# Signalsmith-Audio/signalsmith-stretch

Hardware: AMD Instinct MI355X
Metric: Msamples/sec (in+out) at 48kHz stereo presetDefault (higher is better)
Workload: dtype f32

## Files before the change

signalsmith-stretch_amd/csrc/smst_fft.hip:

```cpp
#include "smst_kernels_common.h"
#include <type_traits>

namespace smst {

template <int SIGN> __device__ __forceinline__ fc mulTwiddle(fc v, fc w) { return fmul<(SIGN > 0)>(v, w); }
template <int SIGN> __device__ __forceinline__ fc addJ(fc a, fc b) { return (SIGN < 0) ? fsubI(a, b) : faddI(a, b); }
template <int SIGN> __device__ __forceinline__ fc subJ(fc a, fc b) { return (SIGN < 0) ? faddI(a, b) : fsubI(a, b); }
template <int SIGN> __device__ __forceinline__ fc mulJ(fc a) { return (SIGN < 0) ? fmake(a.y, -a.x) : fmake(-a.y, a.x); }

template <int SIGN>
__device__ __forceinline__ void dft4(fc &a, fc &b, fc &c, fc &d) {
	const fc apc = fadd(a, c), amc = fsub(a, c), bpd = fadd(b, d), bmd = fsub(b, d);
	a = fadd(apc, bpd);
	b = addJ<SIGN>(amc, bmd);
	c = fsub(apc, bpd);
	d = subJ<SIGN>(amc, bmd);
}
template <int SIGN>
__device__ __forceinline__ void dft4J(fc &a, fc &b, fc &c, fc &d) {
	const fc apc = addJ<SIGN>(a, c), amc = subJ<SIGN>(a, c), bpd = fadd(b, d), bmd = fsub(b, d);
	a = fadd(apc, bpd);
	b = addJ<SIGN>(amc, bmd);
	c = fsub(apc, bpd);
	d = subJ<SIGN>(amc, bmd);
// ... 91 lines not shown
	}
	return reinterpret_cast<float2 *>(src);
}

template <int SIGN>
__device__ __forceinline__ fc mulConst(fc v, float re, float im) {
	const float s = (SIGN < 0) ? -im : im;
	return fmake(v.x*re - v.y*s, v.x*s + v.y*re);
}
template <int SIGN>
__device__ __forceinline__ void dft16(fc (&v)[16]) {
#pragma unroll
	for (int i = 0; i < 4; ++i) dft4<SIGN>(v[i], v[i + 4], v[i + 8], v[i + 12]);
	const float c1 = 0.92387953251128675613f, s1 = 0.38268343236508977173f, h = 0.70710678118654752440f;
	v[1 + 4] = mulConst<SIGN>(v[1 + 4], c1, s1);
	v[1 + 8] = mulConst<SIGN>(v[1 + 8], h, h);
	v[1 + 12] = mulConst<SIGN>(v[1 + 12], s1, c1);
	v[2 + 4] = mulConst<SIGN>(v[2 + 4], h, h);
	v[2 + 12] = mulConst<SIGN>(v[2 + 12], -h, h);
	v[3 + 4] = mulConst<SIGN>(v[3 + 4], s1, c1);
	v[3 + 8] = mulConst<SIGN>(v[3 + 8], -h, h);
	v[3 + 12] = mulConst<SIGN>(v[3 + 12], -c1, -s1);
#pragma unroll
	for (int e = 0; e < 4; ++e) {
		if (e == 2) dft4J<SIGN>(v[4*e], v[4*e + 1], v[4*e + 2], v[4*e + 3]);
		else dft4<SIGN>(v[4*e], v[4*e + 1], v[4*e + 2], v[4*e + 3]);
	}
}
template <int SIGN, int RA, int N>
__device__ __forceinline__ void dftPow2(fc (&v)[N], int base, int stride) {
	if constexpr (RA == 2) {
		const fc a = v[base], b = v[base + stride];
		v[base] = fadd(a, b);
		v[base + stride] = fsub(a, b);
	} else if constexpr (RA == 4) {
		dft4<SIGN>(v[base], v[base + stride], v[base + 2*stride], v[base + 3*stride]);
	} else {
		static_assert(RA == 8, "radix 2, 4 or 8");
		fc e0 = v[base], e1 = v[base + 2*stride], e2 = v[base + 4*stride], e3 = v[base + 6*stride];
		fc o0 = v[base + stride], o1 = v[base + 3*stride], o2 = v[base + 5*stride], o3 = v[base + 7*stride];
		dft4<SIGN>(e0, e1, e2, e3);
		dft4<SIGN>(o0, o1, o2, o3);
		const float h = 0.70710678118654752440f;
		o1 = mulConst<SIGN>(o1, h, h);
		o3 = mulConst<SIGN>(o3, -h, h);
		v[base] = fadd(e0, o0); v[base + 4*stride] = fsub(e0, o0);
		v[base + stride] = fadd(e1, o1); v[base + 5*stride] = fsub(e1, o1);
		v[base + 2*stride] = addJ<SIGN>(e2, o2); v[base + 6*stride] = subJ<SIGN>(e2, o2);
		v[base + 3*stride] = fadd(e3, o3); v[base + 7*stride] = fsub(e3, o3);
	}
}
template <int R3> struct LastStage {
	static constexpr int G = (R3%3 == 0) ? 3 : 5;
	static constexpr int RA = R3/G;
	static_assert(R3%G == 0 && (RA == 2 || RA == 4 || RA == 8), "last stage: {2,4,8} x {3,5} points");
};
template <int SIGN, int R3>
__device__ __forceinline__ void dftLast(fc (&v)[R3]) {
	constexpr int G = LastStage<R3>::G, RA = LastStage<R3>::RA;
#pragma unroll
	for (int i = 0; i < G; ++i) dftPow2<SIGN, RA>(v, i, G);
#pragma unroll
	for (int i = 1; i < G; ++i) {
#pragma unroll
		for (int e = 1; e < RA; ++e) {
			const float ang = 6.28318530717958647692f*float(i*e)/float(R3);
			v[i + G*e] = mulConst<SIGN>(v[i + G*e], __builtin_cosf(ang), __builtin_sinf(ang));
		}
	}
#pragma unroll
	for (int e = 0; e < RA; ++e) {
		if constexpr (G == 3) dft3<SIGN>(v[G*e], v[G*e + 1], v[G*e + 2]);
		else dft5<SIGN>(v[G*e], v[G*e + 1], v[G*e + 2], v[G*e + 3 < R3 ? G*e + 3 : 0], v[G*e + 4 < R3 ? G*e + 4 : 0]);
	}
}

struct BlockSync { __device__ __forceinline__ void operator()() const { __syncthreads(); } };
struct NoHook { __device__ __forceinline__ void operator()() const {} };
struct NoArrival { __device__ __forceinline__ fc operator()(fc v, int) const { return v; } };
template <int FRAMES> struct FrameSet { fc f[FRAMES]; };
struct StageTwiddles { float4 w[8]; };
struct TwiddlesFromTable {};
template <int SIGN, int R3, bool LEAN, int ROUNDS = 0, int FRAMES = 1, typename Load, typename Prep, typename Store, typename Sync = BlockSync, typename LastRead = NoHook,
          typename Requested = NoHook, typename FirstWritten = NoHook, typename Arrived = NoArrival, typename TwRegs = TwiddlesFromTable>
__device__ __forceinline__ void fftFast(float2 *lds2, const float4 *__restrict__ twA, const float4 *__restrict__ twB, Load load, Prep prep, Store store,
                                        const int t = threadIdx.x, Sync sync = Sync(), LastRead lastRead = LastRead(), Requested requested = Requested(),
                                        FirstWritten firstWritten = FirstWritten(), Arrived arrived = Arrived(), TwRegs twRegs = TwRegs()) {
	static_assert(FRAMES == 1 || FRAMES == 2, "one frame, or two in lockstep");
	constexpr int MA = 16*R3, BUF = 17*MA;
	constexpr bool TW_REGS = std::is_same<TwRegs, StageTwiddles>::value;
	static_assert(!(TW_REGS && LEAN), "the lean tables have no register form");
	fc *lds = reinterpret_cast<fc *>(lds2);
	auto prepOf = [&](int j, int idx, int f) { if constexpr (FRAMES == 1) return prep(j, idx); else return prep(j, idx, f); };
	auto storeOf = [&](int j, fc u, auto r, int idx, int f) { if constexpr (FRAMES == 1) store(j, u, r, idx); else store(j, u, r, idx, f); };
	fc v[FRAMES][16];
	if (t < MA) {
#pragma unroll
		for (int k = 0; k < 16; ++k) {
			if constexpr (FRAMES == 1) v[0][k] = load(t + MA*k, k);
			else {
				const FrameSet<FRAMES> both = load(t + MA*k, k);
#pragma unroll
				for (int f = 0; f < FRAMES; ++f) v[f][k] = both.f[f];
			}
		}
	}
	requested();
	if (t < MA) {
#pragma unroll
		for (int f = 0; f < FRAMES; ++f) {
#pragma unroll
			for (int k = 0; k < 16; ++k) {
				if constexpr (FRAMES == 1) v[f][k] = arrived(v[f][k], t + MA*k);
				else v[f][k] = arrived(v[f][k], t + MA*k, k, f);
			}
		}
		fc w[16];
		if constexpr (LEAN) {
			const float4 a = twA[t], b = twA[MA + t], c = twA[2*MA + t];
			w[1] = fmake(a.x, a.y); w[2] = fmake(a.z, a.w); w[3] = fmake(b.x, b.y); w[4] = fmake(b.z, b.w);
			w[8] = fmake(c.x, c.y); w[12] = fmake(c.z, c.w);
#pragma unroll
			for (int hi = 4; hi <= 12; hi += 4) {
#pragma unroll
				for (int lo = 1; lo < 4; ++lo) w[hi + lo] = fmul<false>(w[hi], w[lo]);
			}
		} else {
			float4 wA[8];
#pragma unroll
			for (int i = 0; i < 8; ++i) {
				if constexpr (TW_REGS) wA[i] = twRegs.w[i];
				else wA[i] = twA[i*MA + t];
			}
#pragma unroll
			for (int n = 1; n < 16; ++n) {
				const float4 pr = wA[(n - 1) >> 1];
				w[n] = ((n - 1) & 1) ? fmake(pr.z, pr.w) : fmake(pr.x, pr.y);
			}
		}
#pragma unroll
		for (int f = 0; f < FRAMES; ++f) dft16<SIGN>(v[f]);
#pragma unroll
		for (int f = 0; f < FRAMES; ++f) {
#pragma unroll
			for (int pos = 0; pos < 16; ++pos) {
				const int n = (pos >> 2) + 4*(pos & 3);
				lds[f*BUF + 17*t + n] = n > 0 ? mulTwiddle<SIGN>(v[f][pos], w[n]) : v[f][pos];
			}
		}
	}
	firstWritten();
	sync();
	const int p = t >> 4, q0 = t & 15;
	if (t < MA) {
#pragma unroll
		for (int f = 0; f < FRAMES; ++f) {
#pragma unroll
			for (int k = 0; k < 16; ++k) v[f][k] = lds[f*BUF + q0 + 17*(p + R3*k)];
		}
	}
	sync();
	if (t < MA) {
		float4 wB[8];
#pragma unroll
		for (int i = 0; i < 8; ++i) wB[i] = twB[i*R3 + p];
#pragma unroll
		for (int f = 0; f < FRAMES; ++f) dft16<SIGN>(v[f]);
#pragma unroll
		for (int f = 0; f < FRAMES; ++f) {
#pragma unroll
			for (int pos = 0; pos < 16; ++pos) {
				const int n = (pos >> 2) + 4*(pos & 3);
				fc val = v[f][pos];
				if (n > 0) {
					const float4 pr = wB[(n - 1) >> 1];
					val = mulTwiddle<SIGN>(val, ((n - 1) & 1) ? fmake(pr.z, pr.w) : fmake(pr.x, pr.y));
				}
				lds[f*BUF + q0 + 256*p + 16*n] = val;
			}
		}
	}
	sync();
	if (t < 256) {
		constexpr int G = LastStage<R3>::G, RA = LastStage<R3>::RA;
		fc u[FRAMES][R3];
#pragma unroll
		for (int f = 0; f < FRAMES; ++f) {
#pragma unroll
			for (int k = 0; k < R3; ++k) u[f][k] = lds[f*BUF + t + 256*k];
		}
		lastRead();
		constexpr int CHUNK = ROUNDS ? R3/ROUNDS : (R3 <= 12 ? R3 : (R3 == 24 ? 6 : 5));
		decltype(prepOf(0, 0, 0)) ready[FRAMES][CHUNK];
#pragma unroll
		for (int f = 0; f < FRAMES; ++f) {
#pragma unroll
			for (int i = 0; i < CHUNK; ++i) {
				const int e = i/G, c = i - G*e;
				ready[f][i] = prepOf(t + 256*(e + RA*c), e + RA*c, f);
			}
		}
#pragma unroll
		for (int f = 0; f < FRAMES; ++f) dftLast<SIGN, R3>(u[f]);
#pragma unroll
		for (int f = 0; f < FRAMES; ++f) {
#pragma unroll
			for (int p0 = 0; p0 < R3; p0 += CHUNK) {
				if (p0 > 0) {
#pragma unroll
					for (int i = 0; i < CHUNK; ++i) {
						const int pos = p0 + i, e = pos/G, c = pos - G*e;
						if (pos < R3) ready[f][i] = prepOf(t + 256*(e + RA*c), e + RA*c, f);
					}
				}
#pragma unroll
				for (int i = 0; i < CHUNK; ++i) {
					const int pos = p0 + i, e = pos/G, c = pos - G*e;
					if (pos < R3) storeOf(t + 256*(e + RA*c), u[f][pos], ready[f][i], e + RA*c, f);
				}
			}
		}
	}
}

constexpr int fastBlockThreads(int R3) { return 16*R3 > 256 ? 16*R3 : 256; }

__device__ __forceinline__ bool hopWantsAnalysis(const HopDesc &hd, int which) {
	return (hd.flags & HOP_ACTIVE) && (hd.flags & HOP_NEW_SPECTRUM) && !(hd.flags & HOP_PREANALYSED) && (!which || (hd.flags & HOP_REANALYSE_PREV));
}

// ... 14 lines not shown
	if (slot > 0) r = make_float2(fmaf(xi, w.z, r.x), fmaf(xi, w.w, r.y));
	return r;
}
__device__ __forceinline__ float2 analysisSamples(const float *x0, const float *x1, int m, int slot) {
	return make_float2(slot < 15 ? x0[m] : 0.f, slot > 0 ? x1[m] : 0.f);
}
__device__ __forceinline__ float2 analysisElement(float4 w, const float *x0, const float *x1, int m, int slot) {
	const float2 x = analysisSamples(x0, x1, m, slot);
	return analysisElement(w, x.x, x.y, slot);
}
__device__ __forceinline__ fc leanModulation(float2 hb, int k, int per) {
	const float ang = 3.14159265358979323846f*float(k)/float(per);
	return fmulExpr(fpack(hb), fmake(__builtin_cosf(ang), -__builtin_sinf(ang)));
}
__device__ __forceinline__ void storeWindowed(float *dst, int m, fc u, fc tw, float wRe, float wIm, int B, int H) {
	const int halfB = B/2;
	const fc v = fmulc(u, tw);
	if (m < B - halfB) dst[m + halfB] = (2*v.x)*wRe;
	if (m >= H - halfB) dst[m - H + halfB] = (2*v.y)*wIm;
}
__device__ __forceinline__ void storeWindowed(float *dst, int m, fc u, float4 r, int B, int H) {
	storeWindowed(dst, m, u, fmake(r.x, r.y), r.z, r.w, B, H);
}

template <int R3, bool LEAN>
__global__ __launch_bounds__(fastBlockThreads(R3)) __attribute__((amdgpu_waves_per_eu(4, 4))) void kAnalyseFast(DevBatch d, IoArgs io, int sBase, int hopBase, int lateOnly) {
	extern __shared__ __attribute__((aligned(16))) unsigned char smemRaw[];
	float2 *lds = reinterpret_cast<float2 *>(smemRaw);
	const BlockCoord bc = xcdAwareBlock();
	const int k = bc.x;
	const int c = bc.y >> 1;
	const int which = bc.y & 1;
	const int s = bc.s;
	const HopDesc hd = d.hops[(size_t)(sBase + s)*d.hopStride + hopBase + k];
	if (!hopWantsAnalysis(hd, which)) return;
	if (lateOnly && analysisWindowInCall(d.B, d.M, d.I, hd.inputOffset, which, io.inSamples[sBase + s])) return;
	const int B = d.B, H = d.M, halfB = B/2, N = d.N;
	const int base = hd.inputOffset - (which ? d.I : 0) - B;
	const float *x = io.in + (size_t)(sBase + s)*io.inStreamStride + (size_t)c*io.inChannelStride;
	const float *hist = d.hist + ((size_t)(sBase + s)*d.C + c)*(size_t)d.histPitch + d.histBase[d.histCur][sBase + s] + d.histLen;
	const float2 *__restrict__ winA = d.winA, *__restrict__ winB = d.winB;
	float2 *dst = (which ? d.Xprev : d.Xcur) + rowOf(d, s, k, c);
	auto prep = [](int, int) { return 0; };
	auto store = [&](int j, fc u, int, int) { storeHalfBin(dst, j, u, H, N); };
	constexpr int MA = 16*R3;
	const float4 *__restrict__ twA = LEAN ? d.twA6 : d.twA4;
	const float2 *__restrict__ win2 = d.win2;
	const float2 hb = LEAN ? d.halfTw[min((int)threadIdx.x, MA - 1)] : make_float2(0.f, 0.f);
	if (base >= 0 && H - halfB == MA && B - halfB == 15*MA) {
		const float *x0 = x + base + halfB, *x1 = x + base - H + halfB;
		const float4 *__restrict__ win4 = d.win4;
		fftFast<-1, R3, LEAN>(lds, twA, d.twB4,
			[&](int m, int slot) {
				if constexpr (LEAN) {
					const float2 w = win2[m];
					float2 z = make_float2(0.f, 0.f);
					if (slot < 15) z.x = x0[m]*w.x;
					if (slot > 0) z.y = x1[m]*w.y;
					return fmul<false>(fpack(z), leanModulation(hb, slot, 32));
				} else {
					return fpack(analysisElement(win4[m], x0, x1, m, slot));
				}
			}, prep, store);
		return;
	}
	fftFast<-1, R3, LEAN>(lds, twA, d.twB4,
		[&](int m, int slot) {
			float xr = 0, xi = 0;
			if (m < B - halfB) { int src = base + m + halfB; xr = (src >= 0) ? x[src] : hist[src]; }
			if (m >= H - halfB) { int src = base + m - H + halfB; xi = (src >= 0) ? x[src] : hist[src]; }
			if constexpr (LEAN) {
				const float2 w = win2[m];
				return fmul<false>(fmake(xr*w.x, xi*w.y), leanModulation(hb, slot, 32));
			} else {
				const float2 a = winA[m], b = winB[m];
				return fmake(fmaf(xi, b.x, xr*a.x), fmaf(xi, b.y, xr*a.y));
			}
		}, prep, store);
}

struct TeamSync {
	volatile int *word;
	int *generation;
	__device__ __forceinline__ void operator()() const {
		asm volatile("" ::: "memory");
		__builtin_amdgcn_wave_barrier();
		if ((threadIdx.x & 63) == 0) (void)__hip_atomic_fetch_add(const_cast<int *>(word), 1, __ATOMIC_RELAXED, __HIP_MEMORY_SCOPE_WORKGROUP);
		*generation += 4;
		while (__hip_atomic_load(const_cast<int *>(word), __ATOMIC_RELAXED, __HIP_MEMORY_SCOPE_WORKGROUP) < *generation) __builtin_amdgcn_s_sleep(1);
		__builtin_amdgcn_wave_barrier();
		asm volatile("" ::: "memory");
	}
};
template <int R3, int TEAMS, int FRAMES = 1>
struct TeamWorkgroup {
	static_assert(16*R3 <= 256, "a team is 256 threads");
	static constexpr int MA = 16*R3, H = 256*R3;
	float4 *table, *twA, *twB;
	float2 *lds;
	int team, t;
	volatile int *word;
	int generation = 0;
	__device__ __forceinline__ TeamWorkgroup(unsigned char *smem, const DevBatch &d, const float4 *__restrict__ source) {
		team = __builtin_amdgcn_readfirstlane(threadIdx.x >> 8);
		t = threadIdx.x & 255;
		table = reinterpret_cast<float4 *>(smem);
		twA = table + H;
		twB = twA + (FRAMES == 1 ? 8*MA : 0);
		lds = reinterpret_cast<float2 *>(twB + 8*R3) + (size_t)team*FRAMES*(H + H/16);
		volatile int *words = reinterpret_cast<volatile int *>(reinterpret_cast<float2 *>(twB + 8*R3) + (size_t)TEAMS*FRAMES*(H + H/16));
		for (int i = threadIdx.x; i < H; i += blockDim.x) table[i] = source[i];
		if constexpr (FRAMES == 1) {
			for (int i = threadIdx.x; i < 8*MA; i += blockDim.x) twA[i] = d.twA4[i];
		} else {
			twA = nullptr;
		}
		for (int i = threadIdx.x; i < 8*R3; i += blockDim.x) twB[i] = d.twB4[i];
		if (threadIdx.x < 16) words[threadIdx.x] = 0;
		__syncthreads();
		word = words + team;
	}
	TeamWorkgroup(const TeamWorkgroup &) = delete;
	__device__ __forceinline__ TeamSync sync() { return TeamSync{word, &generation}; }
};

template <int R3, int TEAMS, bool EXACT>
__global__ __launch_bounds__(256*TEAMS) void kAnalyseTeams(DevBatch d, IoArgs io, const HopDesc *__restrict__ hopTable, int sBase, int hopBase, int tileHops, int nStreams) {
	extern __shared__ __attribute__((aligned(16))) unsigned char smemRaw[];
	constexpr int MA = 16*R3, H = 256*R3, N = 2*H;
	const int B = EXACT ? 480*R3 : d.B, halfB = B/2;
	const int total = tileHops*2*d.C*nStreams;
	TeamWorkgroup<R3, TEAMS> wg(smemRaw, d, d.win4);
	const TeamSync sync = wg.sync();
	const int t = wg.t, tA = t < MA ? t : 0;
	const int stride = gridDim.x*TEAMS;
	for (int lin = blockIdx.x + gridDim.x*wg.team; lin < total; lin += stride) {
		const BlockCoord bc = xcdAwareCoord(lin, tileHops, 2*d.C, nStreams);
		const HopDesc hd = hopTable[(size_t)(sBase + bc.s)*d.hopStride + hopBase + bc.x];
		const int c = bc.y >> 1, which = bc.y & 1;
		if (!hopWantsAnalysis(hd, which) || !analysisWindowInCall(B, H, d.I, hd.inputOffset, which, io.inSamples[sBase + bc.s])) continue;
		const int base = hd.inputOffset - (which ? d.I : 0) - B;
		const float *x = io.in + (size_t)(sBase + bc.s)*io.inStreamStride + (size_t)c*io.inChannelStride;
		const float *x0 = x + base + halfB, *x1 = x + base - H + halfB;
		float2 *dst = (which ? d.Xprev : d.Xcur) + rowOf(d, bc.s, bc.x, c);
		fftFast<-1, R3, false>(wg.lds, wg.twA, wg.twB,
			[&](int m, int slot) { return fpack(analysisElement(wg.table[tA + MA*slot], x0, x1, m, slot)); },
			[](int, int) { return 0; },
			[&](int j, fc u, int, int) { storeHalfBin(dst, j, u, H, N); }, t, sync);
		sync();
	}
}

template <int R3, bool EXACT, bool TWIST>
__global__ __launch_bounds__(512) __attribute__((amdgpu_waves_per_eu(2, 2))) void kAnalyseTeamPairs(DevBatch d, IoArgs io, const HopDesc *__restrict__ hopTable, const int *__restrict__ inSamples, int sBase, int hopBase, int tileHops, int nStreams) {
	extern __shared__ __attribute__((aligned(16))) unsigned char smemRaw[];
	constexpr int TEAMS = 2, MA = 16*R3, H = 256*R3, N = 2*H;
	const int B = EXACT ? 480*R3 : d.B, halfB = B/2;
	const int jobs = tileHops*2*d.C;
	const int passes = (jobs + 1)/2, total = passes*nStreams;
	static_assert((H + 8*R3)*sizeof(float4) + TEAMS*2*(H + H/16)*sizeof(float2) + 64 <= 160*1024, "the window, the second-stage twiddles, four transform buffers and the barrier words fit a CU's LDS (155,200 bytes at R3 = 12)");
	TeamWorkgroup<R3, TEAMS, 2> wg(smemRaw, d, d.win4);
	const TeamSync sync = wg.sync();
	const int t = wg.t, tA = t < MA ? t : 0;
	StageTwiddles twA;
#pragma unroll
	for (int i = 0; i < 8; ++i) twA.w[i] = d.twA4[i*MA + tA];
	float2 rotOf[TWIST ? R3 : 1];
	if constexpr (TWIST) {
#pragma unroll
		for (int i = 0; i < R3; ++i) rotOf[i] = d.rot[halfBinIndex(t + 256*i, H, N)];
	}
	const int stride = gridDim.x*TEAMS, rowPasses = TWIST ? tileHops : (tileHops + 1)/2;
	const int turn = 8*((((rowPasses - stride/8)%(2*rowPasses)) + 2*rowPasses)%(2*rowPasses));
	const int place = blockIdx.x + gridDim.x*wg.team;
	for (int round = 0; round*stride < total; ++round) {
		const int lin = round*stride + (place + round*turn)%stride;
		if (lin >= total) continue;
		const BlockCoord pc = xcdAwareCoord(lin, passes, 1, nStreams);
		const int nIn = inSamples[sBase + pc.s];
		HopDesc hd[2];
		BlockCoord bc[2];
		bool have[2];
#pragma unroll
		for (int f = 0; f < 2; ++f) {
			const int job = 2*pc.x + f;
			have[f] = job < jobs;
			const int j = have[f] ? job : 2*pc.x;
			if constexpr (TWIST) {
				const int c = pc.x/tileHops;
				have[f] = true;
				bc[f].y = 2*c + f;
				bc[f].x = pc.x - c*tileHops;
			} else {
				bc[f].y = j/tileHops;
				bc[f].x = j - bc[f].y*tileHops;
			}
			bc[f].s = pc.s;
			hd[f] = hopTable[(size_t)(sBase + pc.s)*d.hopStride + hopBase + bc[f].x];
		}
		const float *x0[2], *x1[2];
		float2 *dst[2];
		bool on[2];
#pragma unroll
		for (int f = 0; f < 2; ++f) {
			const int c = bc[f].y >> 1, which = bc[f].y & 1;
			const bool wanted = hopWantsAnalysis(hd[f], which), inCall = analysisWindowInCall(B, H, d.I, hd[f].inputOffset, which, nIn);
			on[f] = have[f] & wanted & inCall;
			const int base = hd[f].inputOffset - (which ? d.I : 0) - B;
			const float *x = io.in + (size_t)(sBase + pc.s)*io.inStreamStride + (size_t)c*io.inChannelStride;
			x0[f] = x + base + halfB;
			x1[f] = x + base - H + halfB;
			dst[f] = (which ? d.Xprev : d.Xcur) + rowOf(d, pc.s, bc[f].x, c);
		}
		if (!on[0] && !on[1]) continue;
		auto prep = [](int, int, int = 0) { return 0; };
		if (on[0] && on[1]) {
			float4 win[16];
			[[maybe_unused]] fc landed[TWIST ? R3 : 1];
			fftFast<-1, R3, false, 0, 2>(wg.lds, nullptr, wg.twB,
				[&](int m, int slot) {
					FrameSet<2> r;
#pragma unroll
					for (int f = 0; f < 2; ++f) r.f[f] = fpack(analysisSamples(x0[f], x1[f], m, slot));
					return r;
				},
				prep, [&](int j, fc u, int, int idx, int f) {
					if constexpr (TWIST) {
						const fc landedValue = fconjIf(u, 2*j >= H);
						float2 *row = dst[f] + halfBinIndex(j, H, N);
						if (f == 0) { landed[idx] = landedValue; *reinterpret_cast<fc *>(row) = landedValue; }
						else *row = prevHopTwist(funpack(landed[idx]), funpack(landedValue), rotOf[idx]);
					} else {
						storeHalfBin(dst[f], j, u, H, N);
					}
				}, t, sync, NoHook(),
				[&]() {
#pragma unroll
					for (int slot = 0; slot < 16; ++slot) win[slot] = wg.table[tA + MA*slot];
					asm volatile("" ::: "memory");
				},
				NoHook(), [&](fc x, int, int slot, int) { return fpack(analysisElement(win[slot], x.x, x.y, slot)); }, twA);
		} else {
			const int f = on[0] ? 0 : 1;
			const float *xa = x0[f], *xb = x1[f];
			float2 *dstOne = dst[f];
			fftFast<-1, R3, false>(wg.lds, nullptr, wg.twB,
				[&](int m, int slot) { return fpack(analysisElement(wg.table[tA + MA*slot], xa, xb, m, slot)); },
				prep, [&](int j, fc u, int, int) { storeHalfBin(dstOne, j, u, H, N); }, t, sync, NoHook(), NoHook(), NoHook(), NoArrival(), twA);
		}
		sync();
	}
}

__global__ __launch_bounds__(256) void kTwistRows(DevBatch d, IoArgs io, int sBase, int hopBase, int teams) {
	const int k = blockIdx.x, c = blockIdx.y, s = blockIdx.z;
	const HopDesc hd = d.hops[(size_t)(sBase + s)*d.hopStride + hopBase + k];
	if (!hopWantsAnalysis(hd, 1)) return;
	const int nIn = io.inSamples[sBase + s];
	if (teams && analysisWindowInCall(d.B, d.M, d.I, hd.inputOffset, 0, nIn) && analysisWindowInCall(d.B, d.M, d.I, hd.inputOffset, 1, nIn)) return;
	const float2 *cur = d.Xcur + rowOf(d, s, k, c);
	float2 *prev = d.Xprev + rowOf(d, s, k, c);
	for (int b = threadIdx.x; b < d.M; b += blockDim.x) prev[b] = prevHopTwist(cur[b], prev[b], d.rot[b]);
}

template <int R3, bool LEAN>
__global__ __launch_bounds__(fastBlockThreads(R3)) void kSynthFast(DevBatch d, int sBase, int hopBase) {
	extern __shared__ __attribute__((aligned(16))) unsigned char smemRaw[];
	float2 *lds = reinterpret_cast<float2 *>(smemRaw);
	const int k = blockIdx.x, c = blockIdx.y, s = blockIdx.z;
	const HopDesc hd = d.hops[(size_t)(sBase + s)*d.hopStride + hopBase + k];
	if (!(hd.flags & HOP_ACTIVE)) return;
	const int B = d.B, H = d.M, N = d.N;
	const float2 *X = d.OUT + rowOf(d, s, k, c);
	float *__restrict__ frame = frameOf(d, s, k, c);
	auto loadBin = [&](int j, int) { return loadHalfBin(X, j, H, N); };
	if constexpr (LEAN) {
		const float2 *__restrict__ win2 = d.win2;
		const float2 hb = d.halfTw[min((int)threadIdx.x, 255)];
		fftFast<+1, R3, true>(lds, d.twA6, d.twB4, loadBin,
			[&](int m, int) { return win2[m]; },
			[&](int m, fc u, float2 w, int j) { storeWindowed(frame, m, u, leanModulation(hb, j, 2*R3), w.x, w.y, B, H); });
	} else {
		const float4 *__restrict__ synTab = d.synTab;
		fftFast<+1, R3, false>(lds, d.twA4, d.twB4, loadBin,
			[&](int m, int) {
				return synTab[m];
			},
			[&](int m, fc u, float4 r, int) { storeWindowed(frame, m, u, r, B, H); });
	}
}

template <int R3, int TEAMS>
__global__ __launch_bounds__(256*TEAMS) void kSynthTeams(DevBatch d, const HopDesc *__restrict__ hopTable, int sBase, int hopBase, int tileHops, int nStreams) {
	extern __shared__ __attribute__((aligned(16))) unsigned char smemRaw[];
	constexpr int H = 256*R3, N = 2*H;
	const int B = d.B;
	const int total = tileHops*d.C*nStreams;
	TeamWorkgroup<R3, TEAMS> wg(smemRaw, d, d.synTab);
	const TeamSync sync = wg.sync();
	const int stride = gridDim.x*TEAMS;
	for (int lin = blockIdx.x + gridDim.x*wg.team; lin < total; lin += stride) {
		const BlockCoord bc = xcdAwareCoord(lin, tileHops, d.C, nStreams);
		const HopDesc hd = hopTable[(size_t)(sBase + bc.s)*d.hopStride + hopBase + bc.x];
		if (!(hd.flags & HOP_ACTIVE)) continue;
		const float2 *X = d.OUT + rowOf(d, bc.s, bc.x, bc.y);
		float *__restrict__ frame = frameOf(d, bc.s, bc.x, bc.y);
		fftFast<+1, R3, false>(wg.lds, wg.twA, wg.twB,
			[&](int j, int) { return loadHalfBin(X, j, H, N); },
			[&](int m, int) { return wg.table[m]; },
			[&](int m, fc u, float4 r, int) { storeWindowed(frame, m, u, r, B, H); }, wg.t, sync);
		sync();
	}
}

__device__ __forceinline__ float carriedSumAt(const DevBatch &d, size_t row, int i) { return i < d.carryLen ? loadCarrySum(d, d.carryCur, row + i) : 0.0f; }
__device__ __forceinline__ float carriedProductAt(const DevBatch &d, const float *__restrict__ carryWpOld, int i) { return i < d.carryLen ? carryWpOld[i] : 1e-30f; }
struct FrameRange { int lo, hi; };
__device__ __forceinline__ FrameRange coveringFrames(int relFirst, int relLast, int B, int I, int hopCount) {
	FrameRange r;
	r.hi = (relLast >= 0) ? relLast/I : -1;
	r.lo = (relFirst - B + 1 > 0) ? (relFirst - B + 1 + I - 1)/I : 0;
	if (r.hi > hopCount - 1) r.hi = hopCount - 1;
	return r;
}
__device__ __forceinline__ float windowProductAt(const DevBatch &d, const EmitDesc &ed, const float *__restrict__ carryWpOld, int i) {
	float wp = carriedProductAt(d, carryWpOld, i);
	if (ed.hopCount > 0) {
		const int rel = ed.nLo + i - ed.firstHopPos - d.delta;
		const FrameRange q = coveringFrames(rel, rel, d.B, d.I, ed.hopCount);
		for (int k = q.lo; k <= q.hi; ++k) wp += d.wprod[rel - k*d.I];
	}
	return wp;
}
// ... 88 lines not shown
		float *outHops = io.out + (size_t)sg*io.outStreamStride + (size_t)c*io.outChannelStride + firstHopPos;
		const float *wpHead = d.wpHead + (size_t)sg*d.wpHeadLen + off;
		auto overlapAdd = [&]() {
			float e[QN][SLOTS];
			int tt = t;
			keepUnconditional(tt);
#pragma unroll
			for (int a = 0; a < QN; ++a) {
#pragma unroll
				for (int slot = 0; slot < SLOTS; ++slot) {
					if (GI && (256*slot >= GI || a*GI + 256*slot >= GB)) continue;
					e[a][slot] = ex[inFrame(a, slot) ? a*I + 256*slot + tt : 0];
				}
			}
#pragma unroll
			for (int a = 0; a < QN; ++a) {
#pragma unroll
				for (int slot = 0; slot < SLOTS; ++slot) {
					if (GI && (256*slot >= GI || a*GI + 256*slot >= GB)) continue;
					keepUnconditional(e[a][slot]);
					acc[a + DQ][slot] = inFrame(a, slot) ? acc[a + DQ][slot] + e[a][slot] : acc[a + DQ][slot];
				}
			}
		};
		auto moveRing = [&]() {
#pragma unroll
			for (int u = 0; u + 1 < NI; ++u) {
#pragma unroll
				for (int slot = 0; slot < SLOTS; ++slot) acc[u][slot] = acc[u + 1][slot];
			}
#pragma unroll
			for (int slot = 0; slot < SLOTS; ++slot) acc[NI - 1][slot] = 0.0f;
		};
		auto productsOf = [&](int q, float (&wp)[SLOTS]) {
#pragma unroll
			for (int slot = 0; slot < SLOTS; ++slot) wp[slot] = steady[slot];
			if (q < NI) {
				Async4 head[SLOTS];
				const float *from = wpHead + q*I;
#pragma unroll
				for (int slot = 0; slot < SLOTS; ++slot) asyncLoad4(head[slot], from + (inInterval(slot) ? 256*slot + t : 0));
				asyncWait<0>();
#pragma unroll
				for (int slot = 0; slot < SLOTS; ++slot) {
					asyncArrived(head[slot]);
					if (inInterval(slot)) wp[slot] = asyncValue(head[slot]);
				}
			}
		};
		auto emitFinal = [&](int q) {
			float wp[SLOTS];
			productsOf(q, wp);
			float *to = outHops + q*I;
#pragma unroll
			for (int slot = 0; slot < SLOTS; ++slot) {
				if (inInterval(slot)) to[256*slot + t] = acc[0][slot]/wp[slot];
			}
			moveRing();
		};
		Async8 next[16];
#pragma unroll
		for (int k = 0; k < 16; ++k) asyncClear(next[k]);
		auto request = [&](int q) {
			const float2 *X = spectra + (unsigned)q*hopPitch;
			if (t < MA) {
#pragma unroll
				for (int k = 0; k < 16; ++k) asyncLoad8(next[k], X + halfBinIndex(t + MA*k, H, N));
			}
		};
		auto landed = [&]() {
			asyncWait<0>();
#pragma unroll
			for (int k = 0; k < 16; ++k) asyncArrived(next[k]);
		};
		request(0);
		landed();
		for (int q = 0; q < cnt; ++q) {
			fftFast<+1, R3, false, 2>(lds, wg.twA, wg.twB,
				[&](int, int k) { return fpack(asyncValue(next[k])); },
				[&](int m, int) { return wg.table[m]; },
				[&](int m, fc u, float4 r, int) { storeWindowed(ex, m, u, r, B, H); }, t, sync, sync,
				[&]() {
					if (q > 0) overlapAdd();
					sync();
				},
				[&]() {
					if (q > 0) emitFinal(q - 1);
					request(q + 1 < cnt ? q + 1 : q);
				},
				[&](fc v, int j) { return fconjIf(v, 2*j >= H); });
			sync();
			landed();
		}
		overlapAdd();
		sync();
		int sgE = sg, cE = c;
		keepUnconditional(sgE);
		keepUnconditional(cE);
		const SynthEmitEdge e = synthEmitEdge(d, io, __builtin_amdgcn_readfirstlane(sgE), __builtin_amdgcn_readfirstlane(cE), tileIndex);
		auto emitEdge = [&](int q) {
			float wp[SLOTS];
			productsOf(q, wp);
			const int n0 = firstHopPos + q*I;
#pragma unroll
			for (int slot = 0; slot < SLOTS; ++slot) {
				if (inInterval(slot)) synthEmitPlace(d, e, n0 + 256*slot + t, acc[0][slot], wp[slot]);
			}
			moveRing();
		};
		emitEdge(cnt - 1);
		const bool trailing = SPLIT && firstHopPos + cnt*I < e.ed.nHi;
		if (trailing) emitEdge(cnt);
		const int n0 = firstHopPos + (cnt + (trailing ? 1 : 0))*I;
#pragma unroll
		for (int u = 0; u < NI; ++u) {
#pragma unroll
			for (int slot = 0; slot < SLOTS; ++slot) {
				if (inInterval(slot)) synthEmitPlace(d, e, n0 + u*I + 256*slot + t, acc[u][slot], 1.0f);
			}
		}
	}
}

__global__ __launch_bounds__(256) void kEnergy(DevBatch d, IoArgs io, int sBase, float *__restrict__ energyOut) {
	const int s = blockIdx.x, part = blockIdx.y, parts = gridDim.y;
	if (part == 0 && (int)threadIdx.x >= parts && (int)threadIdx.x < kEnergyParts) energyOut[(size_t)(sBase + s)*kEnergyParts + threadIdx.x] = 0.0f;
	const int n = io.inSamples[sBase + s];
	const int lo = (int)((long long)n*part/parts), hi = (int)((long long)n*(part + 1)/parts);
	float acc = 0;
	for (int c = 0; c < d.C; ++c) {
		const float *x = io.in + (size_t)(sBase + s)*io.inStreamStride + (size_t)c*io.inChannelStride;
		for (int i = lo + threadIdx.x; i < hi; i += blockDim.x) {
			float v = x[i];
			acc += v*v;
		}
	}
	extern __shared__ __attribute__((aligned(16))) unsigned char smemRaw[];
	float *red = reinterpret_cast<float *>(smemRaw);
	red[threadIdx.x] = acc;
	__syncthreads();
	for (int w = 128; w > 0; w >>= 1) {
		if ((int)threadIdx.x < w) red[threadIdx.x] += red[threadIdx.x + w];
		__syncthreads();
	}
	if (threadIdx.x == 0) energyOut[(size_t)(sBase + s)*kEnergyParts + part] = red[0];
}

template <bool BIG>
__global__ __launch_bounds__(256) void kAnalyse(DevBatch d, IoArgs io, int sBase, int hopBase) {
	extern __shared__ __attribute__((aligned(16))) unsigned char smemRaw[];
	float2 *bufA = reinterpret_cast<float2 *>(smemRaw);
	float2 *bufB = bufA + d.M;

	const BlockCoord bc = xcdAwareBlock();
	const int k = bc.x;
	const int c = bc.y >> 1;
	const int which = bc.y & 1;
	const int s = bc.s;
	const HopDesc hd = d.hops[(size_t)(sBase + s)*d.hopStride + hopBase + k];
	if (!hopWantsAnalysis(hd, which)) return;

	const int B = d.B, H = d.M, halfB = B/2;
	const int base = hd.inputOffset - (which ? d.I : 0) - B;
	const float *x = io.in + (size_t)(sBase + s)*io.inStreamStride + (size_t)c*io.inChannelStride;
	const float *hist = d.hist + ((size_t)(sBase + s)*d.C + c)*(size_t)d.histPitch + d.histBase[d.histCur][sBase + s];
	const float *__restrict__ win = d.window;
	float2 *dst = (which ? d.Xprev : d.Xcur) + rowOf(d, s, k, c);
	if (BIG) bufB = dst;

	for (int m = threadIdx.x; m < H; m += blockDim.x) {
		float re = 0, im = 0;
		if (m < B - halfB) {
			int i = m + halfB;
			int src = base + i;
			float v = (src >= 0) ? x[src] : hist[d.histLen + src];
// ... 88 lines not shown
				sum[0] += f[k].x; sum[1] += f[k].y; sum[2] += f[k].z; sum[3] += f[k].w;
				wp[0] += w[k].x; wp[1] += w[k].y; wp[2] += w[k].z; wp[3] += w[k].w;
			} else if (q <= qHi) {
				const float *frame = frameOf(d, s, q, c);
#pragma unroll
				for (int j = 0; j < 4; ++j) {
					const int idx = idx0 + j;
					if (idx >= 0 && idx < B) { sum[j] += frame[idx]; wp[j] += d.wprod[idx]; }
				}
			}
		}
		for (int q = qLo + KMAX; q <= qHi; ++q) {
			const int idx0 = rel0 - q*I;
			const float *frame = frameOf(d, s, q, c);
#pragma unroll
			for (int j = 0; j < 4; ++j) {
				const int idx = idx0 + j;
				if (idx >= 0 && idx < B) { sum[j] += frame[idx]; wp[j] += d.wprod[idx]; }
			}
		}
	}
	float *out = io.out + (size_t)sg*io.outStreamStride + (size_t)c*io.outChannelStride + ed.nLo;
	if (i0 + 3 < span) {
		*reinterpret_cast<float4 *>(out + i0) = make_float4(sum[0]/wp[0], sum[1]/wp[1], sum[2]/wp[2], sum[3]/wp[3]);
	} else {
#pragma unroll
		for (int j = 0; j < 4; ++j) {
			const int i = i0 + j;
			if (i < span) {
				out[i] = sum[j]/wp[j];
			} else if (i < total) {
				storeCarrySum(d, d.carryCur ^ 1, carryRow + (i - span), sum[j]);
				if (c == 0) d.carryWp[d.carryCur ^ 1][carryWpRow(d, sg) + (i - span)] = wp[j];
			}
		}
	}
}

__global__ __launch_bounds__(256) void kEmitCarried(DevBatch d, IoArgs io) {
	const int sg = blockIdx.x;
	const EmitDesc ed = d.emit[(size_t)sg*d.emitStride];
	const int span = ed.nHi - ed.nLo, from = d.carryBase[d.carryCur][sg];
	const float *wpRow = d.carryWp[d.carryCur] + carryWpRow(d, sg) + from;
	for (int c = 0; c < d.C; ++c) {
		const size_t row = carrySumRow(d, sg, c) + from;
		float *out = io.out + (size_t)sg*io.outStreamStride + (size_t)c*io.outChannelStride + ed.nLo;
		for (int i = threadIdx.x; i < span; i += blockDim.x) {
			out[i] = carriedSumAt(d, row, i)/carriedProductAt(d, wpRow, i);
		}
	}
	__syncthreads();
	if (threadIdx.x == 0) d.carryBase[d.carryCur][sg] = from + span;
}

void launchEnergy(const DevBatch &d, const IoArgs &io, int sBase, int nStreams, int maxSamples, float *energyOut, hipStream_t st) {
	const int parts = std::max(1, std::min(kEnergyParts, maxSamples/1024));
	hipLaunchKernelGGL(kEnergy, dim3(nStreams, parts), dim3(256), 256*sizeof(float), st, d, io, sBase, energyOut);
}
template <int... R3S, typename F>
static bool withR3(int M, F f) { return M%256 == 0 && withInt<R3S...>(M/256, f); }
template <typename F> static bool withFastR3(int M, F f) { return withR3<10, 12, 20, 24>(M, f); }
template <typename F> static bool withTeamR3(int M, F f) { return withR3<10, 12>(M, f); }
static size_t fastLdsBytes(int M) { return ((size_t)M + M/16)*sizeof(float2); }
static size_t teamLdsBytes(int M, int teams, int frames = 1) {
	const size_t twA = frames == 1 ? M/2 : 0;
	return ((size_t)M + twA + M/32)*sizeof(float4) + teams*frames*fastLdsBytes(M) + 64;
}
static bool fastApplies(const DevBatch &d) { return !d.noFastFft && isFastSize(d.M); }
static bool teamsAvailable(const DevBatch &d) { return fastApplies(d) && withTeamR3(d.M, [](auto) {}) && d.fftTeams && !d.fftLean; }
static bool teamsApply(const DevBatch &d, int jobs) { return teamsAvailable(d) && (d.fftTeams == 2 || jobs >= 6*d.teamsGrid); }
static bool analysePairsApply(const DevBatch &d) { return d.analysePairs != 0; }
static int pairWorkgroups(const DevBatch &d, int passes) {
	return std::max(8, std::min((passes + 1)/2/8*8, d.teamsGrid));
}
static int teamsWorkgroups(const DevBatch &d, int jobs) {
	return std::max(8, std::min((jobs + 2)/3/8*8, d.teamsGrid));
}
constexpr int synthEmitQN(int R3) { return R3 == 10 ? 3 : 4; }
constexpr int synthEmitSlots(int R3) { return R3 == 10 ? 8 : 6; }

bool analyseTwistApplies(const DevBatch &d, int nStreams, int tileHops) { return teamsApply(d, tileHops*d.C*2*nStreams) && analysePairsApply(d); }

void launchAnalyse(const DevBatch &d, const IoArgs &io, int sBase, int nStreams, int hopBase, int tileHops, bool anyInCall, bool anyLate, hipStream_t st, bool twisted, int lateHops) {
	const dim3 grid(tileHops, d.C*2, nStreams);
	const int jobs = tileHops*d.C*2*nStreams;
	const bool teams = anyInCall && teamsApply(d, jobs);
	if (teams) {
		const WindowPad pad = windowPad(d.B, d.M);
		const bool pairs = analysePairsApply(d);
		const int passes = (tileHops*d.C*2 + 1)/2*nStreams;
		withTeamR3(d.M, [&](auto r3) { withFlag(pad.lo == 0 && pad.hi == 0, [&](auto exact) {
			if (pairs && twisted) hipLaunchKernelGGL((kAnalyseTeamPairs<r3.value, exact.value, true>), dim3(pairWorkgroups(d, passes)), dim3(512), teamLdsBytes(d.M, 2, 2), st, d, io, d.hops, io.inSamples, sBase, hopBase, tileHops, nStreams);
			else if (pairs) hipLaunchKernelGGL((kAnalyseTeamPairs<r3.value, exact.value, false>), dim3(pairWorkgroups(d, passes)), dim3(512), teamLdsBytes(d.M, 2, 2), st, d, io, d.hops, io.inSamples, sBase, hopBase, tileHops, nStreams);
			else hipLaunchKernelGGL((kAnalyseTeams<r3.value, 3, exact.value>), dim3(teamsWorkgroups(d, jobs)), dim3(768), teamLdsBytes(d.M, 3), st, d, io, d.hops, sBase, hopBase, tileHops, nStreams);
		}); });
		countLaunch(LK_ANALYSE_TEAMS);
		if (pairs) countLaunch(LK_ANALYSE_PAIRS);
		if (pairs && twisted) countLaunch(LK_ANALYSE_TWIST);
		if (!anyLate) return;
	}
	auto twistRows = [&] {
		if (!twisted || lateHops <= 0) return;
		hipLaunchKernelGGL(kTwistRows, dim3(std::min(lateHops, tileHops), d.C, nStreams), dim3(256), 0, st, d, io, sBase, hopBase, teams ? 1 : 0);
		countLaunch(LK_TWIST_ROWS);
	};
	const int lateOnly = teams ? 1 : 0;
	countLaunch(fastApplies(d) ? LK_ANALYSE_FAST : LK_ANALYSE_GENERIC);
	if (!d.noFastFft && withFastR3(d.M, [&](auto r3) { withFlag(d.fftLean != 0, [&](auto lean) {
			hipLaunchKernelGGL((kAnalyseFast<r3.value, lean.value>), grid, dim3(fastBlockThreads(r3.value)), fastLdsBytes(d.M), st, d, io, sBase, hopBase, lateOnly);
		}); })) { twistRows(); return; }
	size_t lds = 2*(size_t)d.M*sizeof(float2);
	if (fftNeedsScratch(d.M)) hipLaunchKernelGGL(kAnalyse<true>, grid, dim3(256), lds/2, st, d, io, sBase, hopBase);
	else hipLaunchKernelGGL(kAnalyse<false>, grid, dim3(256), lds, st, d, io, sBase, hopBase);
	twistRows();
}
void launchSynth(const DevBatch &d, int sBase, int nStreams, int hopBase, int tileHops, hipStream_t st) {
	const dim3 grid(tileHops, d.C, nStreams);
	const int jobs = tileHops*d.C*nStreams;
	if (teamsApply(d, jobs)) {
		withTeamR3(d.M, [&](auto r3) {
			hipLaunchKernelGGL((kSynthTeams<r3.value, 3>), dim3(teamsWorkgroups(d, jobs)), dim3(768), teamLdsBytes(d.M, 3), st, d, d.hops, sBase, hopBase, tileHops, nStreams);
		});
		countLaunch(LK_SYNTH_TEAMS);
		return;
	}
	countLaunch(fastApplies(d) ? LK_SYNTH_FAST : LK_SYNTH_GENERIC);
	if (!d.noFastFft && withFastR3(d.M, [&](auto r3) { withFlag(d.fftLean != 0, [&](auto lean) {
			hipLaunchKernelGGL((kSynthFast<r3.value, lean.value>), grid, dim3(fastBlockThreads(r3.value)), fastLdsBytes(d.M), st, d, sBase, hopBase);
		}); })) return;
	size_t lds = 2*(size_t)d.M*sizeof(float2);
	if (fftNeedsScratch(d.M)) hipLaunchKernelGGL(kSynth<true>, grid, dim3(256), lds/2, st, d, sBase, hopBase);
	else hipLaunchKernelGGL(kSynth<false>, grid, dim3(256), lds, st, d, sBase, hopBase);
}
bool synthEmitApplies(const DevBatch &d, int nStreams, int tileHops) {
	if (!teamsAvailable(d) || !d.synthEmit) return false;
	if (!(d.delta == 0 || d.delta == d.I)) return false;
	const int QN = synthEmitQN(d.M/256), SLOTS = synthEmitSlots(d.M/256);
	if (QN*d.I < d.B || d.I > 256*SLOTS || d.B > d.N) return false;
	if ((QN + 2)*d.I > d.wpHeadLen) return false;
	return d.synthEmit == 2 || (tileHops >= 8 && nStreams*d.C >= 64);
}
void launchEmitProducts(const DevBatch &d, int sBase, int nStreams, int tileIndex, hipStream_t st) {
	hipLaunchKernelGGL(kEmitProducts, dim3(divUp(d.wpHeadLen + d.carryLen, 256), nStreams), dim3(256), 0, st, d, sBase, tileIndex);
}
template <int GI, int GB> struct SynthEmitGeometry { static constexpr int interval = GI, block = GB, slots = (GI + 255)/256; };
template <int R3, typename F>
static void withSynthEmitGeometry(const DevBatch &d, F f) {
	using Slots = std::integral_constant<int, synthEmitSlots(R3)>;
	auto is = [&](auto g) { return d.I == g.interval && d.B == g.block && (f(g, std::integral_constant<int, g.slots>()), true); };
	if constexpr (R3 == 12) { if (is(SynthEmitGeometry<1440, 5760>()) || is(SynthEmitGeometry<1323, 5292>())) return; }
	if constexpr (R3 == 10) { if (is(SynthEmitGeometry<1920, 4800>()) || is(SynthEmitGeometry<1764, 4410>())) return; }
	f(SynthEmitGeometry<0, 0>(), Slots());
}
void launchSynthEmit(const DevBatch &d, const IoArgs &io, int sBase, int nStreams, int tileIndex, hipStream_t st) {
	const int items = nStreams*d.C;
	const int wgs = std::min(divUp(items, 2), d.teamsGrid);
	withTeamR3(d.M, [&](auto r3) { withFlag(d.delta != 0, [&](auto split) { withSynthEmitGeometry<r3.value>(d, [&](auto g, auto slots) {
		hipLaunchKernelGGL((kSynthEmitTeams<r3.value, synthEmitQN(r3.value), slots.value, split.value, g.interval, g.block>), dim3(wgs), dim3(512), teamLdsBytes(d.M, 2), st, d, io, sBase, tileIndex, nStreams);
	}); }); });
	countLaunch(LK_SYNTH_EMIT);
}
void launchEmit(const DevBatch &d, const IoArgs &io, int sBase, int nStreams, int tileIndex, int maxSpan, hipStream_t st) {
	const dim3 grid(divUp(divUp(maxSpan + d.carryLen, 4), 256), d.C, nStreams);
	const int covering = divUp(d.B + 3, d.I);
	if (covering <= 3) hipLaunchKernelGGL(kEmit<3>, grid, dim3(256), 0, st, d, io, sBase, tileIndex);
	else if (covering <= 4) hipLaunchKernelGGL(kEmit<4>, grid, dim3(256), 0, st, d, io, sBase, tileIndex);
	else if (covering <= 5) hipLaunchKernelGGL(kEmit<5>, grid, dim3(256), 0, st, d, io, sBase, tileIndex);
	else hipLaunchKernelGGL(kEmit<6>, grid, dim3(256), 0, st, d, io, sBase, tileIndex);
}
// ... 7 lines not shown
```

signalsmith-stretch_amd/csrc/smst_kernels_common.h:

```cpp
#pragma once
#include <hip/hip_runtime.h>
#include <atomic>
#include <cstring>
#include <type_traits>
#include "smst_device.h"
#include <smst_complex.h>
#include <smst_fft_complex.h>
#include <smst_async.h>


#ifdef SMST_EXPERIMENTS
#define SMST_SKIP_PRODUCER_MATH(d) ((d).debugMode == 1)
#define SMST_CONSUMER_ONLY_ACKNOWLEDGES(d) ((d).debugMode == 2)
#else
#define SMST_SKIP_PRODUCER_MATH(d) false
#define SMST_CONSUMER_ONLY_ACKNOWLEDGES(d) false
#endif


namespace smst {

__device__ __forceinline__ float cnorm(float2 a) { return __fadd_rn(__fmul_rn(a.x, a.x), __fmul_rn(a.y, a.y)); }
__device__ __forceinline__ float2 cscale(float2 a, float s) { return make_float2(a.x*s, a.y*s); }
__device__ __forceinline__ float2 prevHopTwist(float2 in, float2 prev, float2 rot) {
	const float2 Q = cmul(prev, rot);
	return cmul(rot, cmulc(in, Q));
}

struct CarriedOutput {
	const void *base;
	bool half;
	__device__ __forceinline__ float2 operator[](size_t i) const {
		if (half) { const Half2 h = static_cast<const Half2 *>(base)[i]; return make_float2(float(h.x), float(h.y)); }
		return static_cast<const float2 *>(base)[i];
	}
};
__device__ __forceinline__ CarriedOutput carriedOutput(const DevBatch &d, int sGlobal) {
	const size_t row = ((size_t)sGlobal*d.C)*(size_t)d.M;
	CarriedOutput r;
	r.half = d.halfState != 0;
	r.base = r.half ? static_cast<const void *>(reinterpret_cast<const Half2 *>(d.stOut) + row) : static_cast<const void *>(d.stOut + row);
	return r;
}
__device__ __forceinline__ void storeCarriedOutput(const DevBatch &d, size_t i, float2 v) {
	if (d.halfState) { Half2 h; h.x = half_t(v.x); h.y = half_t(v.y); reinterpret_cast<Half2 *>(d.stOut)[i] = h; }
	else d.stOut[i] = v;
}
__device__ __forceinline__ float loadCarriedEnergy(const DevBatch &d, size_t i) {
	if (d.halfState) { const float a = float(reinterpret_cast<const half_t *>(d.stEnergy)[i]); return a*a; }
	return d.stEnergy[i];
}
__device__ __forceinline__ void storeCarriedEnergy(const DevBatch &d, size_t i, float e) {
	if (d.halfState) reinterpret_cast<half_t *>(d.stEnergy)[i] = half_t(__builtin_amdgcn_sqrtf(e));
	else d.stEnergy[i] = e;
}
__device__ __forceinline__ size_t carrySumRow(const DevBatch &d, int sg, int c) { return ((size_t)sg*d.C + c)*(size_t)d.carryPitch; }
__device__ __forceinline__ size_t carryWpRow(const DevBatch &d, int sg) { return (size_t)sg*(size_t)d.carryPitch; }
__device__ __forceinline__ float loadCarrySum(const DevBatch &d, int buf, size_t i) {
	return d.halfState ? float(reinterpret_cast<const half_t *>(d.carrySum[buf])[i]) : d.carrySum[buf][i];
}
__device__ __forceinline__ void storeCarrySum(const DevBatch &d, int buf, size_t i, float v) {
	if (d.halfState) reinterpret_cast<half_t *>(d.carrySum[buf])[i] = half_t(v);
	else d.carrySum[buf][i] = v;
}

__device__ __forceinline__ size_t rowOf(const DevBatch &d, int s, int k, int c) {
	return ((size_t)((size_t)s*d.T + k)*d.C + c)*(size_t)d.Mp;
}
__device__ __forceinline__ float *frameOf(const DevBatch &d, int s, int k, int c) {
	return d.frames + ((size_t)((size_t)s*d.T + k)*d.C + c)*(size_t)d.B;
}
__device__ __forceinline__ size_t stateRow(const DevBatch &d, int sGlobal, int c) {
	return ((size_t)sGlobal*d.C + c)*(size_t)d.M;
}

struct BlockCoord { int x, y, s; };
__device__ __forceinline__ BlockCoord xcdAwareCoord(int lin, int gx, int gy, int S) {
	const int n = gx*gy;
	const int g = lin/(8*n), rest = lin - g*8*n;
	BlockCoord r;
	int idx;
	if (8*g + 8 <= S) { r.s = 8*g + (rest & 7); idx = rest >> 3; }
	else { r.s = 8*g + rest/n; idx = rest%n; }
	r.x = idx%gx;
	r.y = idx/gx;
	return r;
}
__device__ __forceinline__ BlockCoord xcdAwareBlock() {
	return xcdAwareCoord(blockIdx.x + gridDim.x*(blockIdx.y + gridDim.y*blockIdx.z), gridDim.x, gridDim.y, gridDim.z);
}

constexpr unsigned kLcgModulus = 2147483647u, kLcgMultiplier = 16807u;
__device__ __forceinline__ unsigned lcgMulMod(unsigned a, unsigned b) {
	const unsigned long long p = (unsigned long long)a*b;
	unsigned r = unsigned(p & kLcgModulus) + unsigned(p >> 31);
	r = (r & kLcgModulus) + (r >> 31);
	return r >= kLcgModulus ? r - kLcgModulus : r;
}
__device__ __forceinline__ float engineDraw(const DevBatch &d, unsigned state, int index, float lo, float hi) {
	const unsigned x = lcgMulMod(state, d.lcgPow[index]);
	float u = float(x - 1u)*4.656612873077392578125e-10f;
	if (u >= 1.0f) u = 0.999999940395355224609375f;
	return __fadd_rn(__fmul_rn(u, hi - lo), lo);
}

static inline int divUp(int a, int b) { return (a + b - 1)/b; }
void countLaunch(LaunchKind k);
template <int... VALUES, typename F>
static bool withInt(int v, F f) { return ((v == VALUES && (f(std::integral_constant<int, VALUES>()), true)) || ...); }
// ... 17 lines not shown
```

Before: 52990.

## Split team barriers into arrive/wait and defer twist stores after FFT

Splits the team spin barrier into separate arrive and wait phases so independent work (twiddle multiplication, overlap-add, landing) can run between the arrival and the wait. The FFT first-write stage gains a hook that applies twiddles before waiting, then writes LDS afterward. In the paired analysis kernel, the second frame's twist is deferred and computed in batched passes after the FFT, with per-pass addresses computed from the thread index, and the trailing sync per pass is dropped. The analysis grid is also shrunk to the late-hop count when teams apply. This risks ordering hazards if the removed syncs were protecting LDS reuse.

```diff
diff --git a/signalsmith-stretch_amd/csrc/smst_fft.hip b/signalsmith-stretch_amd/csrc/smst_fft.hip
--- a/signalsmith-stretch_amd/csrc/smst_fft.hip
+++ b/signalsmith-stretch_amd/csrc/smst_fft.hip
@@ -197,13 +197,16 @@
 struct StageTwiddles { float4 w[8]; };
 struct TwiddlesFromTable {};
 template <int SIGN, int R3, bool LEAN, int ROUNDS = 0, int FRAMES = 1, typename Load, typename Prep, typename Store, typename Sync = BlockSync, typename LastRead = NoHook,
-          typename Requested = NoHook, typename FirstWritten = NoHook, typename Arrived = NoArrival, typename TwRegs = TwiddlesFromTable>
+          typename Requested = NoHook, typename FirstWritten = NoHook, typename Arrived = NoArrival, typename TwRegs = TwiddlesFromTable,
+          typename BeforeFirstWrite = NoHook>
 __device__ __forceinline__ void fftFast(float2 *lds2, const float4 *__restrict__ twA, const float4 *__restrict__ twB, Load load, Prep prep, Store store,
                                         const int t = threadIdx.x, Sync sync = Sync(), LastRead lastRead = LastRead(), Requested requested = Requested(),
-                                        FirstWritten firstWritten = FirstWritten(), Arrived arrived = Arrived(), TwRegs twRegs = TwRegs()) {
+                                        FirstWritten firstWritten = FirstWritten(), Arrived arrived = Arrived(), TwRegs twRegs = TwRegs(),
+                                        BeforeFirstWrite beforeFirstWrite = BeforeFirstWrite()) {
 	static_assert(FRAMES == 1 || FRAMES == 2, "one frame, or two in lockstep");
 	constexpr int MA = 16*R3, BUF = 17*MA;
 	constexpr bool TW_REGS = std::is_same<TwRegs, StageTwiddles>::value;
+	constexpr bool SPLIT_FIRST_WRITE = !std::is_same<BeforeFirstWrite, NoHook>::value;
 	static_assert(!(TW_REGS && LEAN), "the lean tables have no register form");
 	fc *lds = reinterpret_cast<fc *>(lds2);
 	auto prepOf = [&](int j, int idx, int f) { if constexpr (FRAMES == 1) return prep(j, idx); else return prep(j, idx, f); };
@@ -255,12 +258,37 @@
 		}
 #pragma unroll
 		for (int f = 0; f < FRAMES; ++f) dft16<SIGN>(v[f]);
-#pragma unroll
-		for (int f = 0; f < FRAMES; ++f) {
-#pragma unroll
-			for (int pos = 0; pos < 16; ++pos) {
-				const int n = (pos >> 2) + 4*(pos & 3);
-				lds[f*BUF + 17*t + n] = n > 0 ? mulTwiddle<SIGN>(v[f][pos], w[n]) : v[f][pos];
+		if constexpr (!SPLIT_FIRST_WRITE) {
+#pragma unroll
+			for (int f = 0; f < FRAMES; ++f) {
+#pragma unroll
+				for (int pos = 0; pos < 16; ++pos) {
+					const int n = (pos >> 2) + 4*(pos & 3);
+					lds[f*BUF + 17*t + n] = n > 0 ? mulTwiddle<SIGN>(v[f][pos], w[n]) : v[f][pos];
+				}
+			}
+		} else {
+#pragma unroll
+			for (int f = 0; f < FRAMES; ++f) {
+#pragma unroll
+				for (int pos = 0; pos < 16; ++pos) {
+					const int n = (pos >> 2) + 4*(pos & 3);
+					if (n > 0) v[f][pos] = mulTwiddle<SIGN>(v[f][pos], w[n]);
+				}
+			}
+		}
+	}
+	if constexpr (SPLIT_FIRST_WRITE) {
+		beforeFirstWrite();
+		if (t < MA) {
+#pragma unroll
+			for (int f = 0; f < FRAMES; ++f) {
+#pragma unroll
+				for (int pos = 0; pos < 16; ++pos) {
+					const int n = (pos >> 2) + 4*(pos & 3);
+					lds[f*BUF + 17*t + n] = v[f][pos];
+					asm volatile("");
+				}
 			}
 		}
 	}
@@ -441,11 +469,14 @@
 struct TeamSync {
 	volatile int *word;
 	int *generation;
-	__device__ __forceinline__ void operator()() const {
+	__device__ __forceinline__ void operator()() const { arrive(); wait(); }
+	__device__ __forceinline__ void arrive() const {
 		asm volatile("" ::: "memory");
 		__builtin_amdgcn_wave_barrier();
 		if ((threadIdx.x & 63) == 0) (void)__hip_atomic_fetch_add(const_cast<int *>(word), 1, __ATOMIC_RELAXED, __HIP_MEMORY_SCOPE_WORKGROUP);
 		*generation += 4;
+	}
+	__device__ __forceinline__ void wait() const {
 		while (__hip_atomic_load(const_cast<int *>(word), __ATOMIC_RELAXED, __HIP_MEMORY_SCOPE_WORKGROUP) < *generation) __builtin_amdgcn_s_sleep(1);
 		__builtin_amdgcn_wave_barrier();
 		asm volatile("" ::: "memory");
@@ -514,6 +545,7 @@
 __global__ __launch_bounds__(512) __attribute__((amdgpu_waves_per_eu(2, 2))) void kAnalyseTeamPairs(DevBatch d, IoArgs io, const HopDesc *__restrict__ hopTable, const int *__restrict__ inSamples, int sBase, int hopBase, int tileHops, int nStreams) {
 	extern __shared__ __attribute__((aligned(16))) unsigned char smemRaw[];
 	constexpr int TEAMS = 2, MA = 16*R3, H = 256*R3, N = 2*H;
+	constexpr bool ADDR_PER_PASS = TWIST && EXACT && R3 == 12;
 	const int B = EXACT ? 480*R3 : d.B, halfB = B/2;
 	const int jobs = tileHops*2*d.C;
 	const int passes = (jobs + 1)/2, total = passes*nStreams;
@@ -573,9 +605,13 @@
 		}
 		if (!on[0] && !on[1]) continue;
 		auto prep = [](int, int, int = 0) { return 0; };
+		auto arrive = [&]() { sync.arrive(); };
+		auto wait = [&]() { sync.wait(); };
 		if (on[0] && on[1]) {
 			float4 win[16];
 			[[maybe_unused]] fc landed[TWIST ? R3 : 1];
+			[[maybe_unused]] fc earlier[TWIST ? R3 : 1];
+			int ts = t;
 			fftFast<-1, R3, false, 0, 2>(wg.lds, nullptr, wg.twB,
 				[&](int m, int slot) {
 					FrameSet<2> r;
@@ -586,28 +622,41 @@
 				prep, [&](int j, fc u, int, int idx, int f) {
 					if constexpr (TWIST) {
 						const fc landedValue = fconjIf(u, 2*j >= H);
-						float2 *row = dst[f] + halfBinIndex(j, H, N);
-						if (f == 0) { landed[idx] = landedValue; *reinterpret_cast<fc *>(row) = landedValue; }
-						else *row = prevHopTwist(funpack(landed[idx]), funpack(landedValue), rotOf[idx]);
+						if (f == 0) { landed[idx] = landedValue; *reinterpret_cast<fc *>(dst[0] + halfBinIndex(ADDR_PER_PASS ? ts + 256*idx : j, H, N)) = landedValue; }
+						else earlier[idx] = landedValue;
 					} else {
 						storeHalfBin(dst[f], j, u, H, N);
 					}
-				}, t, sync, NoHook(),
+				}, t, sync,
+				[&]() {
+					sync.arrive();
+					if constexpr (ADDR_PER_PASS) { keepUnconditional(ts); ts &= 255; }
+				},
 				[&]() {
 #pragma unroll
 					for (int slot = 0; slot < 16; ++slot) win[slot] = wg.table[tA + MA*slot];
 					asm volatile("" ::: "memory");
 				},
-				NoHook(), [&](fc x, int, int slot, int) { return fpack(analysisElement(win[slot], x.x, x.y, slot)); }, twA);
+				NoHook(), [&](fc x, int, int slot, int) { return fpack(analysisElement(win[slot], x.x, x.y, slot)); }, twA, wait);
+			if constexpr (TWIST) {
+				float2 tw[R3];
+#pragma unroll
+				for (int i = 0; i < R3; ++i) tw[i] = prevHopTwistTurned(funpack(earlier[i]), rotOf[i]);
+#pragma unroll
+				for (int i = 0; i < R3; ++i) tw[i] = prevHopTwistAgainst(funpack(landed[i]), tw[i]);
+#pragma unroll
+				for (int i = 0; i < R3; ++i) tw[i] = prevHopTwistTurnedBack(rotOf[i], tw[i]);
+#pragma unroll
+				for (int i = 0; i < R3; ++i) dst[1][halfBinIndex(ts + 256*i, H, N)] = tw[i];
+			}
 		} else {
 			const int f = on[0] ? 0 : 1;
 			const float *xa = x0[f], *xb = x1[f];
 			float2 *dstOne = dst[f];
 			fftFast<-1, R3, false>(wg.lds, nullptr, wg.twB,
 				[&](int m, int slot) { return fpack(analysisElement(wg.table[tA + MA*slot], xa, xb, m, slot)); },
-				prep, [&](int j, fc u, int, int) { storeHalfBin(dstOne, j, u, H, N); }, t, sync, NoHook(), NoHook(), NoHook(), NoArrival(), twA);
-		}
-		sync();
+				prep, [&](int j, fc u, int, int) { storeHalfBin(dstOne, j, u, H, N); }, t, sync, arrive, NoHook(), NoHook(), NoArrival(), twA, wait);
+		}
 	}
 }
 
@@ -862,15 +911,18 @@
 				[&](int m, fc u, float4 r, int) { storeWindowed(ex, m, u, r, B, H); }, t, sync, sync,
 				[&]() {
 					if (q > 0) overlapAdd();
-					sync();
+					sync.arrive();
 				},
 				[&]() {
 					if (q > 0) emitFinal(q - 1);
 					request(q + 1 < cnt ? q + 1 : q);
 				},
-				[&](fc v, int j) { return fconjIf(v, 2*j >= H); });
-			sync();
+				[&](fc v, int j) { return fconjIf(v, 2*j >= H); },
+				TwiddlesFromTable(),
+				[&]() { sync.wait(); });
+			sync.arrive();
 			landed();
+			sync.wait();
 		}
 		overlapAdd();
 		sync();
@@ -1125,9 +1177,9 @@
 bool analyseTwistApplies(const DevBatch &d, int nStreams, int tileHops) { return teamsApply(d, tileHops*d.C*2*nStreams) && analysePairsApply(d); }
 
 void launchAnalyse(const DevBatch &d, const IoArgs &io, int sBase, int nStreams, int hopBase, int tileHops, bool anyInCall, bool anyLate, hipStream_t st, bool twisted, int lateHops) {
-	const dim3 grid(tileHops, d.C*2, nStreams);
 	const int jobs = tileHops*d.C*2*nStreams;
 	const bool teams = anyInCall && teamsApply(d, jobs);
+	const dim3 grid(teams && lateHops > 0 ? std::min(lateHops, tileHops) : tileHops, d.C*2, nStreams);
 	if (teams) {
 		const WindowPad pad = windowPad(d.B, d.M);
 		const bool pairs = analysePairsApply(d);
diff --git a/signalsmith-stretch_amd/csrc/smst_kernels_common.h b/signalsmith-stretch_amd/csrc/smst_kernels_common.h
--- a/signalsmith-stretch_amd/csrc/smst_kernels_common.h
+++ b/signalsmith-stretch_amd/csrc/smst_kernels_common.h
@@ -22,9 +22,11 @@
 
 __device__ __forceinline__ float cnorm(float2 a) { return __fadd_rn(__fmul_rn(a.x, a.x), __fmul_rn(a.y, a.y)); }
 __device__ __forceinline__ float2 cscale(float2 a, float s) { return make_float2(a.x*s, a.y*s); }
+__device__ __forceinline__ float2 prevHopTwistTurned(float2 prev, float2 rot) { return cmul(prev, rot); }
+__device__ __forceinline__ float2 prevHopTwistAgainst(float2 in, float2 Q) { return cmulc(in, Q); }
+__device__ __forceinline__ float2 prevHopTwistTurnedBack(float2 rot, float2 P) { return cmul(rot, P); }
 __device__ __forceinline__ float2 prevHopTwist(float2 in, float2 prev, float2 rot) {
-	const float2 Q = cmul(prev, rot);
-	return cmul(rot, cmulc(in, Q));
+	return prevHopTwistTurnedBack(rot, prevHopTwistAgainst(in, prevHopTwistTurned(prev, rot)));
 }
 
 struct CarriedOutput {
```

New measurement: 53370, median of 6. About the same (+0.7%).
